# arpg/ba

Hardware: AMD Instinct MI355X
Metric: Gauss-Newton iterations/sec (higher is better)
Workload: dtype f64; 1 GPU; BASELINE.json configs[3]: 10000 poses / 1000000 landmarks / 10000000 reprojection residuals, pinhole, LmSize=1, PoseSize=6, Gauss-Newton (no dogleg), 2 anchor poses inactive; poses=10000, landmarks=1000000, residuals=10000000, reduced_system_n=59988, driver=phase calls of the C-ABI (include/ba_hip.h), parallelism=single GPU

## Files before the change

ba_amd/csrc/k_chol.hip:

```cpp
#include "engine.h"
#include <cstdlib>
#include <algorithm>
#include <vector>

namespace bae {

static const int NB = 64;
static const int LDT = NB + 2;

typedef double double4_t __attribute__((ext_vector_type(4)));

__device__ __forceinline__ double readlane_f64(double v, int lane) {
  int lo = __double2loint(v), hi = __double2hiint(v);
  lo = __builtin_amdgcn_readlane(lo, lane);
  hi = __builtin_amdgcn_readlane(hi, lane);
  return __hiloint2double(hi, lo);
}

static const int LDM = 18;

static const int KC2 = 16;
#ifndef BAE_LDK2
#define BAE_LDK2 (KC2 + 2)
#endif
static const int LDK2 = BAE_LDK2;

__device__ __forceinline__ void update_tile_fast(double* __restrict__ A, uint32_t ld, uint32_t i, uint32_t c,
                                                 uint32_t kb0, uint64_t mask, double (*X)[NB][LDK2],
                                                 double (*Y)[NB][LDK2]) {
  const int tid = threadIdx.x, wave = tid >> 6, lane = tid & 63;
  const int li = lane & 15, lk = lane >> 4;
  const int rb = 32 * (wave >> 1), cb = 32 * (wave & 1);
  double* Aic = A + ((size_t)i * NB) * ld + (size_t)c * NB;
  double4_t acc[2][2];
#pragma unroll
  for (int ti = 0; ti < 2; ++ti)
#pragma unroll
    for (int tj = 0; tj < 2; ++tj) acc[ti][tj] = (double4_t){0.0, 0.0, 0.0, 0.0};
  const int sr = tid >> 3, sc = (tid & 7) * 2;
  const double* Xg0 = A + ((size_t)i * NB + sr) * ld + sc;
  const double* Xg1 = Xg0 + (size_t)32 * ld;
  const double* Yg0 = A + ((size_t)c * NB + sr) * ld + sc;
  const double* Yg1 = Yg0 + (size_t)32 * ld;
  double2 px0[2], px1[2], py0[2], py1[2];
  double F0[4], F1[4];
  double4_t cv[2][2];
#define BAE_SB __builtin_amdgcn_sched_barrier(0)
#define BAE_GLOAD(S, K0)                                        \
  {                                                             \
    px0[S] = *reinterpret_cast<const double2*>(Xg0 + (K0));     \
    px1[S] = *reinterpret_cast<const double2*>(Xg1 + (K0));     \
    py0[S] = *reinterpret_cast<const double2*>(Yg0 + (K0));     \
    py1[S] = *reinterpret_cast<const double2*>(Yg1 + (K0));     \
  }
#define BAE_SSTORE(B, S)                                                    \
  {                                                                         \
    X[B][sr][sc] = px0[S].x; X[B][sr][sc + 1] = px0[S].y;                   \
    X[B][sr + 32][sc] = px1[S].x; X[B][sr + 32][sc + 1] = px1[S].y;         \
    Y[B][sr][sc] = py0[S].x; Y[B][sr][sc + 1] = py0[S].y;                   \
    Y[B][sr + 32][sc] = py1[S].x; Y[B][sr + 32][sc + 1] = py1[S].y;         \
  }
#define BAE_LDF(F, B, KS)                                                              \
  {                                                                                    \
    F[0] = X[B][rb + li][4 * (KS) + lk]; F[1] = X[B][rb + 16 + li][4 * (KS) + lk];     \
    F[2] = Y[B][cb + li][4 * (KS) + lk]; F[3] = Y[B][cb + 16 + li][4 * (KS) + lk];     \
  }
#define BAE_MM(F)                                                                    \
  {                                                                                  \
    acc[0][0] = __builtin_amdgcn_mfma_f64_16x16x4f64(F[0], F[2], acc[0][0], 0, 0, 0); \
    acc[0][1] = __builtin_amdgcn_mfma_f64_16x16x4f64(F[0], F[3], acc[0][1], 0, 0, 0); \
    acc[1][0] = __builtin_amdgcn_mfma_f64_16x16x4f64(F[1], F[2], acc[1][0], 0, 0, 0); \
    acc[1][1] = __builtin_amdgcn_mfma_f64_16x16x4f64(F[1], F[3], acc[1][1], 0, 0, 0); \
  }
#define BAE_CHUNK(J, STORE, LOADK, NEXT)                          \
  {                                                               \
    if (STORE) BAE_SSTORE(((J) + 1) & 1, ((J) + 1) & 1);          \
    LOADK;                                                        \
    BAE_SB; BAE_LDF(F1, (J) & 1, 1); BAE_SB; BAE_MM(F0); BAE_SB;  \
    BAE_LDF(F0, (J) & 1, 2); BAE_SB; BAE_MM(F1); BAE_SB;          \
    BAE_LDF(F1, (J) & 1, 3); BAE_SB; BAE_MM(F0); BAE_SB;          \
    __syncthreads(); BAE_SB;                                      \
    if (NEXT) BAE_LDF(F0, ((J) + 1) & 1, 0);                      \
    BAE_SB; BAE_MM(F1); BAE_SB;                                   \
  }
  uint32_t kcur = (kb0 + (uint32_t)__builtin_ctzll(mask)) * NB;
  mask &= mask - 1;
  BAE_GLOAD(0, kcur);
  BAE_GLOAD(1, kcur + KC2);
  BAE_SSTORE(0, 0);
  BAE_GLOAD(0, kcur + 2 * KC2);
  __syncthreads();
  BAE_LDF(F0, 0, 0);
  while (mask) {
    const uint32_t knext = (kb0 + (uint32_t)__builtin_ctzll(mask)) * NB;
    mask &= mask - 1;
    BAE_CHUNK(0, true, BAE_GLOAD(1, kcur + 3 * KC2), true);
    BAE_CHUNK(1, true, BAE_GLOAD(0, knext), true);
    BAE_CHUNK(2, true, BAE_GLOAD(1, knext + KC2), true);
    BAE_CHUNK(3, true, BAE_GLOAD(0, knext + 2 * KC2), true);
    kcur = knext;
  }
  BAE_CHUNK(0, true, BAE_GLOAD(1, kcur + 3 * KC2), true);
  BAE_CHUNK(1, true, , true);
#define BAE_CLOAD                                                                              \
  _Pragma("unroll") for (int ti = 0; ti < 2; ++ti)                                             \
    _Pragma("unroll") for (int tj = 0; tj < 2; ++tj)                                           \
      _Pragma("unroll") for (int reg = 0; reg < 4; ++reg)                                      \
        cv[ti][tj][reg] = Aic[(size_t)(rb + 16 * ti + lk + 4 * reg) * ld + cb + 16 * tj + li];
  BAE_CHUNK(2, true, BAE_CLOAD, true);
#undef BAE_CLOAD
  BAE_CHUNK(3, false, , false);
#undef BAE_SB
#undef BAE_GLOAD
#undef BAE_SSTORE
#undef BAE_LDF
#undef BAE_MM
#undef BAE_CHUNK
  const bool diag = (i == c);
#pragma unroll
  for (int ti = 0; ti < 2; ++ti)
#pragma unroll
    for (int tj = 0; tj < 2; ++tj)
#pragma unroll
      for (int reg = 0; reg < 4; ++reg) {
        const int r = rb + 16 * ti + lk + 4 * reg;
        const int cc = cb + 16 * tj + li;
        if (!diag || cc <= r) Aic[(size_t)r * ld + cc] = cv[ti][tj][reg] - acc[ti][tj][reg];
      }
}

__device__ __forceinline__ void update_tile(double* __restrict__ A, uint32_t ld, uint32_t nblk, uint32_t i,
                                            uint32_t c, uint32_t kb0, uint32_t kb1,
                                            const double* __restrict__ dsgn, const int* __restrict__ colneg,
                                            const uint8_t* __restrict__ nz, double (*X)[NB][LDK2],
                                            double (*Y)[NB][LDK2], uint32_t* klist) {
  const int rows = (i == nblk) ? 1 : NB;
  const int tid = threadIdx.x, wave = tid >> 6, lane = tid & 63;
  const int li = lane & 15, lk = lane >> 4;
  const int rb = 32 * (wave >> 1), cb = 32 * (wave & 1);
  double* Aic = A + ((size_t)i * NB) * ld + (size_t)c * NB;
  double4_t acc[2][2];
#pragma unroll
  for (int ti = 0; ti < 2; ++ti)
#pragma unroll
    for (int tj = 0; tj < 2; ++tj) acc[ti][tj] = (double4_t){0.0, 0.0, 0.0, 0.0};
  const int sr = tid >> 3, sc = (tid & 7) * 2;
  const double* Xg0 = A + ((size_t)i * NB + (sr < rows ? sr : 0)) * ld + sc;
  const double* Xg1 = A + ((size_t)i * NB + (sr + 32 < rows ? sr + 32 : 0)) * ld + sc;
  const double* Yg0 = A + ((size_t)c * NB + sr) * ld + sc;
  const double* Yg1 = Yg0 + (size_t)32 * ld;
  const double xm0 = sr < rows ? 1.0 : 0.0, xm1 = sr + 32 < rows ? 1.0 : 0.0;
#ifndef BAE_NO_FAST
  if (rows == NB && kb1 - kb0 <= 64u) {
    const uint32_t kl = kb0 + (uint32_t)lane;
    bool on = kl < kb1;
    bool neg = false;
    if (on) {
      neg = colneg[kl] != 0;
      if (nz) on = nz[(size_t)i * nblk + kl] && nz[(size_t)c * nblk + kl];
    }
    const uint64_t mask = __ballot(on);
    if (__ballot(neg) == 0) {
      if (mask == 0) return;
      update_tile_fast(A, ld, i, c, kb0, mask, X, Y);
      return;
    }
  }
#endif
  uint32_t nact = 0;
  for (uint32_t kb = kb0; kb < kb1; ++kb) {
    const bool on = !nz || ((i == nblk || nz[(size_t)i * nblk + kb]) && nz[(size_t)c * nblk + kb]);
    if (on) {
      if (threadIdx.x == 0) klist[nact] = kb * NB;
      ++nact;
    }
  }
  if (nact == 0) return;
  __syncthreads();
  const int nchunk = (int)nact * (NB / KC2);
  double2 px0[2], px1[2], py0[2], py1[2], ps[2] = {make_double2(1.0, 1.0), make_double2(1.0, 1.0)};
  bool plain = rows == NB;
  for (uint32_t kb = kb0; kb < kb1; ++kb) plain = plain && (colneg[kb] == 0);
#define BAE_GLOAD(S, CH)                                                          \
  {                                                                               \
    const uint32_t k0_ = klist[(CH) >> 2] + (uint32_t)((CH) & 3) * KC2;           \
    px0[S] = *reinterpret_cast<const double2*>(Xg0 + k0_);                        \
    px1[S] = *reinterpret_cast<const double2*>(Xg1 + k0_);                        \
    py0[S] = *reinterpret_cast<const double2*>(Yg0 + k0_);                        \
    py1[S] = *reinterpret_cast<const double2*>(Yg1 + k0_);                        \
    if (!plain) ps[S] = *reinterpret_cast<const double2*>(dsgn + k0_ + sc);       \
  }
#define BAE_SSTORE(B, S)                                                          \
  if (plain) {                                                                    \
    X[B][sr][sc] = px0[S].x; X[B][sr][sc + 1] = px0[S].y;                         \
    X[B][sr + 32][sc] = px1[S].x; X[B][sr + 32][sc + 1] = px1[S].y;               \
    Y[B][sr][sc] = py0[S].x; Y[B][sr][sc + 1] = py0[S].y;                         \
    Y[B][sr + 32][sc] = py1[S].x; Y[B][sr + 32][sc + 1] = py1[S].y;               \
  } else {                                                                        \
    X[B][sr][sc] = px0[S].x * xm0; X[B][sr][sc + 1] = px0[S].y * xm0;             \
    X[B][sr + 32][sc] = px1[S].x * xm1; X[B][sr + 32][sc + 1] = px1[S].y * xm1;   \
    Y[B][sr][sc] = ps[S].x * py0[S].x; Y[B][sr][sc + 1] = ps[S].y * py0[S].y;     \
    Y[B][sr + 32][sc] = ps[S].x * py1[S].x; Y[B][sr + 32][sc + 1] = ps[S].y * py1[S].y; \
  }
#define BAE_MMA(B)                                                                \
  _Pragma("unroll") for (int ks = 0; ks < KC2 / 4; ++ks) {                        \
    const double a0 = X[B][rb + li][4 * ks + lk];                                 \
    const double a1 = X[B][rb + 16 + li][4 * ks + lk];                            \
    const double b0 = Y[B][cb + li][4 * ks + lk];                                 \
    const double b1 = Y[B][cb + 16 + li][4 * ks + lk];                            \
    acc[0][0] = __builtin_amdgcn_mfma_f64_16x16x4f64(a0, b0, acc[0][0], 0, 0, 0); \
    acc[0][1] = __builtin_amdgcn_mfma_f64_16x16x4f64(a0, b1, acc[0][1], 0, 0, 0); \
    acc[1][0] = __builtin_amdgcn_mfma_f64_16x16x4f64(a1, b0, acc[1][0], 0, 0, 0); \
    acc[1][1] = __builtin_amdgcn_mfma_f64_16x16x4f64(a1, b1, acc[1][1], 0, 0, 0); \
  }
  BAE_GLOAD(0, 0);
  BAE_GLOAD(1, 1);
  BAE_SSTORE(0, 0);
  BAE_GLOAD(0, 2);
  __syncthreads();
  for (int kc = 0; kc + 2 < nchunk; kc += 2) {
    BAE_SSTORE(1, 1);
    if (kc + 3 < nchunk) BAE_GLOAD(1, kc + 3);
    BAE_MMA(0);
    __syncthreads();
    BAE_SSTORE(0, 0);
    if (kc + 4 < nchunk) BAE_GLOAD(0, kc + 4);
    BAE_MMA(1);
    __syncthreads();
  }
  BAE_SSTORE(1, 1);
  double4_t cv[2][2];
#pragma unroll
  for (int ti = 0; ti < 2; ++ti)
#pragma unroll
    for (int tj = 0; tj < 2; ++tj)
#pragma unroll
      for (int reg = 0; reg < 4; ++reg) {
        const int r = rb + 16 * ti + lk + 4 * reg;
        cv[ti][tj][reg] = Aic[(size_t)(r < rows ? r : 0) * ld + cb + 16 * tj + li];
      }
  BAE_MMA(0);
  __syncthreads();
  BAE_MMA(1);
#undef BAE_GLOAD
#undef BAE_SSTORE
#undef BAE_MMA
  const bool diag = (i == c);
#pragma unroll
  for (int ti = 0; ti < 2; ++ti)
#pragma unroll
    for (int tj = 0; tj < 2; ++tj)
#pragma unroll
      for (int reg = 0; reg < 4; ++reg) {
        const int r = rb + 16 * ti + lk + 4 * reg;
        const int cc = cb + 16 * tj + li;
        if (r < rows && (!diag || cc <= r)) Aic[(size_t)r * ld + cc] = cv[ti][tj][reg] - acc[ti][tj][reg];
      }
}

template <bool BULK>
__global__ void __launch_bounds__(256, BULK ? 2 : 4)
k_update2(double* __restrict__ A, uint32_t ld, uint32_t nblk, uint32_t c0, uint32_t kb0,
          uint32_t kb1, const double* __restrict__ dsgn, const int* __restrict__ colneg, int swz,
          const uint8_t* __restrict__ nz, const OwnMap own) {
  __shared__ double X[2][NB][LDK2];
  __shared__ double Y[2][NB][LDK2];
  __shared__ uint32_t klist[32];
  __shared__ double pad_[BULK ? 2432 : 1];
  if (BULK && kb0 == 0xffffffffu) pad_[threadIdx.x] = 0.0;
  if (!BULK) __builtin_amdgcn_s_setprio(2);
  uint32_t c, i;
  if (swz & 1) {
    const uint32_t sbl = (uint32_t)swz >> 8;
    const uint32_t b = blockIdx.x, xcd = b & 7u, slot = b >> 3;
    const uint32_t t = (slot >> (2 * sbl)) * 8u + xcd, within = slot & ((1u << (2 * sbl)) - 1u);
    uint32_t sr = (uint32_t)((sqrt(8.0 * (double)t + 1.0) - 1.0) * 0.5);
    while ((uint64_t)(sr + 1) * (sr + 2) / 2 <= t) ++sr;
    while ((uint64_t)sr * (sr + 1) / 2 > t) --sr;
    const uint32_t sc = t - (uint32_t)((uint64_t)sr * (sr + 1) / 2);
    const uint32_t R = (sr << sbl) + (within >> sbl), C = (sc << sbl) + (within & ((1u << sbl) - 1u));
    if (C > R) return;
    c = c0 + C;
    i = c0 + R;
    if (i > nblk || c >= nblk) return;
  } else {
    c = c0 + blockIdx.y;
    i = c + blockIdx.x;
    if (i > nblk) return;
  }
  if (!own_tile(own, i, c, nblk)) return;
  update_tile(A, ld, nblk, i, c, kb0, kb1, dsgn, colneg, nz, X, Y, klist);
}

static const int NB2 = 128;
#ifdef BAE_TIME128
__device__ unsigned long long* g_t128_buf = nullptr;
__device__ unsigned int g_t128_n = 0;
static const unsigned int T128_CAP = 1u << 21, T128_REC = 6;
#endif
template <bool RECT, bool LIST = false>
__global__ void __launch_bounds__(256, 2)
k_update128(double* __restrict__ A, uint32_t ld, uint32_t nblk, uint32_t c0, uint32_t m2, uint32_t kb0,
            uint32_t kb1, const double* __restrict__ dsgn, const int* __restrict__ colneg, uint32_t sbl,
            const uint8_t* __restrict__ nz, const OwnMap own,
            uint32_t nrow64, uint32_t r0, uint32_t rect_cols) {
  __shared__ double X[2][NB2][LDK2];
  __shared__ double Y[2][NB2][LDK2];
  __shared__ uint32_t klist[32];
  if (blockIdx.x < nrow64) {
    const uint32_t mcols = RECT ? 2 * rect_cols : nblk - c0, y = blockIdx.x / mcols;
    const uint32_t c = c0 + blockIdx.x % mcols, i = nblk - y;
    if (y > ((nblk - r0) & 1u) || c > i || c >= nblk) return;
    if (!own_tile(own, i, c, nblk)) return;
    update_tile(A, ld, nblk, i, c, kb0, kb1, dsgn, colneg, nz, reinterpret_cast<double(*)[NB][LDK2]>(&X[0][0][0]),
                reinterpret_cast<double(*)[NB][LDK2]>(&Y[0][0][0]), klist);
    return;
  }
  const uint32_t b = blockIdx.x - nrow64;
  uint32_t R, C;
  if constexpr (LIST) {
    const uint32_t gb = own.G >> 1, per = gb * gb;
    const uint32_t pr = b / per, within = b - pr * per;
    const uint2* pairs = reinterpret_cast<const uint2*>(((unsigned long long)own.pairs_hi << 32) | own.pairs_lo);
    const uint2 bp = pairs[pr];
    const uint32_t base = c0 / own.G;
    R = (bp.x - base) * gb + within / gb;
    C = (bp.y - base) * gb + within % gb;
    if (C > R || R >= m2) return;
  } else if (RECT) {
    R = b / rect_cols;
    C = b % rect_cols;
    if (R >= m2) return;
  } else {
    const uint32_t xcd = b & 7u, slot = b >> 3;
    const uint32_t t = (slot >> (2 * sbl)) * 8u + xcd, within = slot & ((1u << (2 * sbl)) - 1u);
    uint32_t sr_ = (uint32_t)((sqrt(8.0 * (double)t + 1.0) - 1.0) * 0.5);
    while ((uint64_t)(sr_ + 1) * (sr_ + 2) / 2 <= t) ++sr_;
    while ((uint64_t)sr_ * (sr_ + 1) / 2 > t) --sr_;
    const uint32_t sc_ = t - (uint32_t)((uint64_t)sr_ * (sr_ + 1) / 2);
    R = (sr_ << sbl) + (within >> sbl);
    C = (sc_ << sbl) + (within & ((1u << sbl) - 1u));
    if (C > R || R >= m2) return;
  }
  const uint32_t c = c0 + 2 * C, i = r0 + 2 * R;
  if (!own_tile(own, i, c, nblk)) return;
  const int tid = threadIdx.x, wave = tid >> 6, lane = tid & 63;
  const uint32_t kl = kb0 + (uint32_t)lane;
  bool on = kl < kb1, neg = false;
  if (on) {
    neg = colneg[kl] != 0;
    if (nz)
      on = (nz[(size_t)i * nblk + kl] | nz[(size_t)(i + 1) * nblk + kl]) &&
           (nz[(size_t)c * nblk + kl] | nz[(size_t)(c + 1) * nblk + kl]);
  }
  uint64_t mask = __ballot(on);
  if (mask == 0) return;
  if (__ballot(neg) != 0 || kb1 - kb0 > 64u) {
    double(*X64)[NB][LDK2] = reinterpret_cast<double(*)[NB][LDK2]>(&X[0][0][0]);
    double(*Y64)[NB][LDK2] = reinterpret_cast<double(*)[NB][LDK2]>(&Y[0][0][0]);
    for (uint32_t q = 0; q < 4; ++q) {
      const uint32_t ii = i + (q >> 1), cc = c + (q & 1);
      if (cc > ii) continue;
      __syncthreads();
      update_tile(A, ld, nblk, ii, cc, kb0, kb1, dsgn, colneg, nz, X64, Y64, klist);
    }
    return;
  }
  const bool diag = (i == c);
  const int li = lane & 15, lk = lane >> 4;
  const int rb = 64 * (wave >> 1), cb = 64 * (wave & 1);
  double4_t acc[4][4];
#pragma unroll
  for (int ti = 0; ti < 4; ++ti)
#pragma unroll
    for (int tj = 0; tj < 4; ++tj) acc[ti][tj] = (double4_t){0.0, 0.0, 0.0, 0.0};
  const int sr = tid >> 3, sc = (tid & 7) * 2;
  const double* Xg = A + ((size_t)i * NB + sr) * ld + sc;
  const double* Yg = A + ((size_t)c * NB + sr) * ld + sc;
  const size_t ld32 = (size_t)32 * ld;
  double2 px[4], py[4];
  double FA0[4], FB0[4], FA1[4], FB1[4];
#ifdef BAE_NO_SCHED_PINS_128
#define BAE_SB
#else
#define BAE_SB __builtin_amdgcn_sched_barrier(0)
#endif
#ifndef BAE_KMASK
#define BAE_KMASK 0xffffffffu
#endif
#define BAE_GLOAD(K0)                                                                \
  _Pragma("unroll") for (int u = 0; u < 4; ++u) {                                    \
    px[u] = *reinterpret_cast<const double2*>(Xg + u * ld32 + ((K0) & BAE_KMASK));   \
    py[u] = *reinterpret_cast<const double2*>(Yg + u * ld32 + ((K0) & BAE_KMASK));   \
  }
#define BAE_SSTORE(B)                                                                \
  _Pragma("unroll") for (int u = 0; u < 4; ++u) {                                    \
    X[B][sr + 32 * u][sc] = px[u].x; X[B][sr + 32 * u][sc + 1] = px[u].y;            \
    Y[B][sr + 32 * u][sc] = py[u].x; Y[B][sr + 32 * u][sc + 1] = py[u].y;            \
  }
#define BAE_LDF(FA, FB, B, KS)                                                       \
  _Pragma("unroll") for (int q = 0; q < 4; ++q) {                                    \
    FA[q] = X[B][rb + 16 * q + li][4 * (KS) + lk];                                   \
    FB[q] = Y[B][cb + 16 * q + li][4 * (KS) + lk];                                   \
  }
#define BAE_MM(FA, FB)                                                               \
  _Pragma("unroll") for (int ti = 0; ti < 4; ++ti)                                   \
    _Pragma("unroll") for (int tj = 0; tj < 4; ++tj)                                 \
      acc[ti][tj] = __builtin_amdgcn_mfma_f64_16x16x4f64(FA[ti], FB[tj], acc[ti][tj], 0, 0, 0);
#define BAE_CHUNK(J, STORE, LOADK, NEXT)                                             \
  {                                                                                  \
    if (STORE) BAE_SSTORE(((J) + 1) & 1);                                            \
    LOADK;                                                                           \
    BAE_SB; BAE_LDF(FA1, FB1, (J) & 1, 1); BAE_SB; BAE_MM(FA0, FB0); BAE_SB;         \
    BAE_LDF(FA0, FB0, (J) & 1, 2); BAE_SB; BAE_MM(FA1, FB1); BAE_SB;                 \
    BAE_LDF(FA1, FB1, (J) & 1, 3); BAE_SB; BAE_MM(FA0, FB0); BAE_SB;                 \
    __syncthreads(); BAE_SB;                                                         \
    if (NEXT) BAE_LDF(FA0, FB0, ((J) + 1) & 1, 0);                                   \
    BAE_SB; BAE_MM(FA1, FB1); BAE_SB;                                                \
  }
#ifdef BAE_TIME128
  const unsigned long long tt0 = __builtin_readcyclecounter();
  const unsigned long long tw0 = wall_clock64();
  const int tt_cols = __builtin_popcountll(mask);
#endif
  uint32_t kcur = (kb0 + (uint32_t)__builtin_ctzll(mask)) * NB;
  mask &= mask - 1;
  BAE_GLOAD(kcur);
  BAE_SSTORE(0);
  BAE_GLOAD(kcur + KC2);
  __syncthreads();
  BAE_LDF(FA0, FB0, 0, 0);
#ifdef BAE_TIME128
  const unsigned long long tt1 = __builtin_readcyclecounter();
  const unsigned long long tw1 = wall_clock64();
#endif
  while (mask) {
    const uint32_t knext = (kb0 + (uint32_t)__builtin_ctzll(mask)) * NB;
    mask &= mask - 1;
    BAE_CHUNK(0, true, BAE_GLOAD(kcur + 2 * KC2), true);
    BAE_CHUNK(1, true, BAE_GLOAD(kcur + 3 * KC2), true);
    BAE_CHUNK(2, true, BAE_GLOAD(knext), true);
    BAE_CHUNK(3, true, BAE_GLOAD(knext + KC2), true);
    kcur = knext;
  }
  double* Aic = A + ((size_t)i * NB) * ld + (size_t)c * NB;
  double4_t cva[4], cvb[4];
#define BAE_CLOAD(CV, TI)                                                            \
  _Pragma("unroll") for (int tj = 0; tj < 4; ++tj)                                   \
    _Pragma("unroll") for (int reg = 0; reg < 4; ++reg)                              \
      CV[tj][reg] = Aic[(size_t)(rb + 16 * (TI) + lk + 4 * reg) * ld + cb + 16 * tj + li];
#define BAE_CSTORE(CV, TI)                                                           \
  _Pragma("unroll") for (int tj = 0; tj < 4; ++tj)                                   \
    _Pragma("unroll") for (int reg = 0; reg < 4; ++reg) {                            \
      const int r = rb + 16 * (TI) + lk + 4 * reg;                                   \
      const int cc = cb + 16 * tj + li;                                              \
      if (!diag || cc <= r) Aic[(size_t)r * ld + cc] = CV[tj][reg] - acc[TI][tj][reg]; \
    }
  BAE_CHUNK(0, true, BAE_GLOAD(kcur + 2 * KC2), true);
  BAE_CHUNK(1, true, BAE_GLOAD(kcur + 3 * KC2), true);
  BAE_CHUNK(2, true, , true);
  BAE_CHUNK(3, false, BAE_CLOAD(cva, 0), false);
#ifdef BAE_TIME128
  const unsigned long long tt2 = __builtin_readcyclecounter();
  const unsigned long long tw2 = wall_clock64();
#endif
  if (diag && wave == 1) return;
  BAE_SB;
  BAE_CLOAD(cvb, 1);
  BAE_SB;
  BAE_CSTORE(cva, 0);
  BAE_SB;
  BAE_CLOAD(cva, 2);
  BAE_SB;
  BAE_CSTORE(cvb, 1);
  BAE_SB;
  BAE_CLOAD(cvb, 3);
  BAE_SB;
  BAE_CSTORE(cva, 2);
  BAE_CSTORE(cvb, 3);
#ifdef BAE_TIME128
  if (tid == 0 && (blockIdx.x % 257u) == 100u && !RECT) {
    const unsigned long long tt3 = __builtin_readcyclecounter();
    printf("T128 cols %d prologue %llu loop %llu epilogue %llu per_chunk %llu loop_100MHz %llu\n", tt_cols, tt1 - tt0,
           tt2 - tt1, tt3 - tt2, (tt2 - tt1) / (unsigned long long)(4 * tt_cols), tw2 - tw1);
  }
  if (tid == 0 && !RECT && g_t128_buf) {
    const unsigned int idx = atomicAdd(&g_t128_n, 1u);
    if (idx < T128_CAP) {
      unsigned long long* r = g_t128_buf + (size_t)idx * T128_REC;
      r[0] = tw0; r[1] = tw1; r[2] = tw2; r[3] = wall_clock64();
      r[4] = ((unsigned long long)__builtin_amdgcn_s_getreg(6164) << 32) | (unsigned int)__builtin_amdgcn_s_getreg(63492);
      r[5] = (unsigned long long)blockIdx.x | ((unsigned long long)tt_cols << 32) | ((unsigned long long)kb0 << 40);
    }
  }
#endif
#undef BAE_CLOAD
#undef BAE_CSTORE
#undef BAE_SB
#undef BAE_GLOAD
#undef BAE_SSTORE
#undef BAE_LDF
#undef BAE_MM
#undef BAE_CHUNK
}

static const int NOPV = 40;

struct TileLds {
  double T[NB][LDT];
  double Md[4][16][LDM];
  double dv[NB];
  double sg[NB];
  __attribute__((aligned(16))) double colbuf[2][NB];
  int bad;
  int neg;
};

__device__ __forceinline__ void factor_tile_wave0(TileLds& sh, int lane, const double* __restrict__ floor_tile) {
  const int li = lane & 15, lk = lane >> 4;
  unsigned long long negmask = 0;
#pragma unroll
  for (int pb = 0; pb < 4; ++pb) {
    const int c0 = 16 * pb;
    double p[16];
#pragma unroll
    for (int c = 0; c < 16; ++c) p[c] = (c0 + c <= lane) ? sh.T[lane][c0 + c] : 0.0;
    double sa_prev = 0.0;
    double lb[16];
    double d = readlane_f64(p[0], c0);
#pragma unroll
    for (int j = 0; j < 16; ++j) {
      const int J = c0 + j;
      const int dhi = __double2hiint(d);
      const int sbit = dhi & (int)0x80000000;
      negmask |= (unsigned long long)((unsigned)dhi >> 31) << J;
      const double ad = fabs(d);
#define BAE_UPD(n)                                      \
  {                                                     \
    const int c_ = j + 1 + (n);                         \
    if (j > 0 && c_ < 16) p[c_] -= sa_prev * lb[c_];    \
  }
#define BAE_SB __builtin_amdgcn_sched_barrier(0)
      double y = __builtin_amdgcn_rsq(ad);
      BAE_SB;
      double t = ad * y;
      BAE_SB;
      double h = fma(-t, y, 1.0);
      BAE_UPD(0) BAE_SB;
      double q = fma(0.375, h, 0.5);
      double yh = y * h;
      BAE_UPD(1) BAE_UPD(2) BAE_UPD(3) BAE_SB;
      y = fma(yh, q, y);
      BAE_UPD(4) BAE_UPD(5) BAE_UPD(6) BAE_UPD(7) BAE_UPD(8) BAE_SB;
      const double sa = p[j] * y;
      BAE_UPD(9) BAE_UPD(10) BAE_SB;
      const double l = __hiloint2double(__double2hiint(sa) ^ sbit, __double2loint(sa));
      sh.colbuf[j & 1][lane] = l;
      p[j] = l;
      BAE_UPD(11) BAE_UPD(12) BAE_UPD(13) BAE_UPD(14) BAE_SB;
#pragma unroll
      for (int c = j + 2; c < 16; ++c) lb[c] = sh.colbuf[j & 1][c0 + c];
      BAE_SB;
      if (j < 15) {
        p[j + 1] -= sa * readlane_f64(l, J + 1);
        d = readlane_f64(p[j + 1], J + 1);
      }
      BAE_SB;
#undef BAE_UPD
#undef BAE_SB
      sa_prev = sa;
    }
#pragma unroll
    for (int c = 0; c < 16; ++c) sh.T[lane][c0 + c] = (c0 + c <= lane) ? p[c] : 0.0;
    sh.sg[lane] = ((negmask >> lane) & 1ull) ? -1.0 : 1.0;
    if (pb < 3) {
      double la[4][3], nb[4][3];
#pragma unroll
      for (int ks = 0; ks < 4; ++ks) {
        const int k = c0 + 4 * ks + lk;
        const double sk = -sh.sg[k];
#pragma unroll
        for (int b = pb + 1; b < 4; ++b) {
          la[ks][b - 1] = sh.T[16 * b + li][k];
          nb[ks][b - 1] = sk * la[ks][b - 1];
        }
      }
#pragma unroll
      for (int rbk = pb + 1; rbk < 4; ++rbk)
#pragma unroll
        for (int cbk = pb + 1; cbk <= rbk; ++cbk) {
          double4_t acc;
#pragma unroll
          for (int reg = 0; reg < 4; ++reg) acc[reg] = sh.T[16 * rbk + lk + 4 * reg][16 * cbk + li];
#pragma unroll
          for (int ks = 0; ks < 4; ++ks)
            acc = __builtin_amdgcn_mfma_f64_16x16x4f64(la[ks][rbk - 1], nb[ks][cbk - 1], acc, 0, 0, 0);
#pragma unroll
          for (int reg = 0; reg < 4; ++reg) sh.T[16 * rbk + lk + 4 * reg][16 * cbk + li] = acc[reg];
        }
    }
  }
  if (lane == 0) sh.neg = negmask != 0 ? 1 : 0;
  {
    const double q = sh.T[lane][lane];
    if (!(q > 0.0 && q < 1e150)) sh.bad = 1;
    if (floor_tile && q * q < floor_tile[lane]) sh.bad = 1;
    sh.dv[lane] = 1.0 / q;
  }
  {
    const int base = 16 * lk, c = li;
    double sacc[16];
#pragma unroll
    for (int r = 0; r < 16; ++r) sacc[r] = (r == c) ? 1.0 : 0.0;
#pragma unroll
    for (int k = 0; k < 16; ++k) {
      const double xk = sacc[k] * sh.dv[base + k];
      sacc[k] = xk;
#pragma unroll
      for (int r = k + 1; r < 16; ++r) sacc[r] -= sh.T[base + r][base + k] * xk;
    }
#pragma unroll
    for (int r = 0; r < 16; ++r) sh.Md[lk][r][c] = sacc[r];
  }
}

__device__ __forceinline__ double subst_operand(const TileLds& sh, int v, int li, int lk, bool sgn) {
  if (v < 16) {
    const int c = v >> 2, ks = v & 3;
    return (sgn ? sh.sg[16 * c + li] : 1.0) * sh.Md[c][li][4 * ks + lk];
  }
  const int pi = (v - 16) >> 2, ks = v & 3;
  const int c = pi == 0 ? 1 : (pi < 3 ? 2 : 3);
  const int k = pi == 0 ? 0 : (pi < 3 ? pi - 1 : pi - 3);
  const int kk = 16 * k + 4 * ks + lk;
  return -(sgn ? sh.sg[kk] : 1.0) * sh.T[16 * c + li][kk];
}

__device__ __forceinline__ void subst_rows(double4_t R[4], const double op[NOPV]) {
#pragma unroll
  for (int c = 0; c < 4; ++c) {
    double4_t Zc = (double4_t){0.0, 0.0, 0.0, 0.0};
#pragma unroll
    for (int ks = 0; ks < 4; ++ks) Zc = __builtin_amdgcn_mfma_f64_16x16x4f64(op[4 * c + ks], R[c][ks], Zc, 0, 0, 0);
#pragma unroll
    for (int c2 = c + 1; c2 < 4; ++c2) {
      const int pi = (c2 == 1 ? 0 : (c2 == 2 ? 1 : 3)) + c;
#pragma unroll
      for (int ks = 0; ks < 4; ++ks)
        R[c2] = __builtin_amdgcn_mfma_f64_16x16x4f64(op[16 + 4 * pi + ks], Zc[ks], R[c2], 0, 0, 0);
    }
    R[c] = Zc;
  }
}

template <bool FACTOR>
__global__ void __launch_bounds__(256, 2)
k_step_update(double* __restrict__ A, uint32_t ld, uint32_t nblk, uint32_t c0, uint32_t kb0,
              uint32_t kb1, double* __restrict__ dsgn, double* __restrict__ opbuf,
              int* __restrict__ colneg, int* __restrict__ status, const uint8_t* __restrict__ nz,
              uint32_t row_end, const uint32_t* __restrict__ rowlist) {
  struct UpdLds { double X[2][NB][LDK2]; double Y[2][NB][LDK2]; };
  __shared__ uint32_t klist[32];
  constexpr size_t kLds = sizeof(TileLds) > sizeof(UpdLds) ? sizeof(TileLds) : sizeof(UpdLds);
  __shared__ __attribute__((aligned(16))) unsigned char smem[kLds];
  UpdLds& u = *reinterpret_cast<UpdLds*>(smem);
  TileLds& sh = *reinterpret_cast<TileLds*>(smem);
  __builtin_amdgcn_s_setprio(2);
  const uint32_t c = c0 + blockIdx.y;
  const uint32_t i = rowlist ? rowlist[blockIdx.x] : c + blockIdx.x;
  if (i > nblk || i >= row_end || i < c) return;
  const bool special = FACTOR && (i == c0 && c == c0);
  if (!special) {
    update_tile(A, ld, nblk, i, c, kb0, kb1, dsgn, colneg, nz, u.X, u.Y, klist);
    return;
  }
  const int rows = (i == nblk) ? 1 : NB;
  const int tid = threadIdx.x, wave = tid >> 6, lane = tid & 63;
  const int li = lane & 15, lk = lane >> 4;
  const int rb = 32 * (wave >> 1), cb = 32 * (wave & 1);
  uint32_t nact = 0;
  for (uint32_t kb = kb0; kb < kb1; ++kb) {
    const bool on = !nz || ((i == nblk || nz[(size_t)i * nblk + kb]) && nz[(size_t)c * nblk + kb]);
    if (on) {
      if (tid == 0) klist[nact] = kb * NB;
      ++nact;
    }
  }
  __syncthreads();
  double* Aic = A + ((size_t)i * NB) * ld + (size_t)c * NB;
  double4_t acc[2][2];
#pragma unroll
  for (int ti = 0; ti < 2; ++ti)
#pragma unroll
    for (int tj = 0; tj < 2; ++tj)
#pragma unroll
      for (int reg = 0; reg < 4; ++reg) {
        const int r = rb + 16 * ti + lk + 4 * reg;
        acc[ti][tj][reg] = Aic[(size_t)(r < rows ? r : 0) * ld + cb + 16 * tj + li];
      }
  const int nchunk = (int)nact * (NB / KC2);
  if (nchunk > 0) {
    const int sr = tid >> 3, sc = (tid & 7) * 2;
    const double* Xg0 = A + ((size_t)i * NB + (sr < rows ? sr : 0)) * ld + sc;
    const double* Xg1 = A + ((size_t)i * NB + (sr + 32 < rows ? sr + 32 : 0)) * ld + sc;
    const double* Yg0 = A + ((size_t)c * NB + sr) * ld + sc;
    const double* Yg1 = Yg0 + (size_t)32 * ld;
    const double xm0 = sr < rows ? 1.0 : 0.0, xm1 = sr + 32 < rows ? 1.0 : 0.0;
    double2 px0, px1, py0, py1, ps;
    auto gload = [&](uint32_t k0) {
      px0 = *reinterpret_cast<const double2*>(Xg0 + k0);
      px1 = *reinterpret_cast<const double2*>(Xg1 + k0);
      py0 = *reinterpret_cast<const double2*>(Yg0 + k0);
      py1 = *reinterpret_cast<const double2*>(Yg1 + k0);
      ps = *reinterpret_cast<const double2*>(dsgn + k0 + sc);
    };
    auto sstore = [&](int b) {
      u.X[b][sr][sc] = px0.x * xm0; u.X[b][sr][sc + 1] = px0.y * xm0;
      u.X[b][sr + 32][sc] = px1.x * xm1; u.X[b][sr + 32][sc + 1] = px1.y * xm1;
      u.Y[b][sr][sc] = -ps.x * py0.x; u.Y[b][sr][sc + 1] = -ps.y * py0.y;
      u.Y[b][sr + 32][sc] = -ps.x * py1.x; u.Y[b][sr + 32][sc + 1] = -ps.y * py1.y;
    };
    auto kof = [&](int ch) { return klist[ch >> 2] + (uint32_t)(ch & 3) * KC2; };
    gload(kof(0));
    sstore(0);
    if (nchunk > 1) gload(kof(1));
    __syncthreads();
    for (int kc = 0; kc < nchunk; ++kc) {
      const int b = kc & 1;
      if (kc + 1 < nchunk) sstore(b ^ 1);
      if (kc + 2 < nchunk) gload(kof(kc + 2));
#pragma unroll
      for (int ks = 0; ks < KC2 / 4; ++ks) {
        const double a0 = u.X[b][rb + li][4 * ks + lk];
        const double a1 = u.X[b][rb + 16 + li][4 * ks + lk];
        const double b0 = u.Y[b][cb + li][4 * ks + lk];
        const double b1 = u.Y[b][cb + 16 + li][4 * ks + lk];
        acc[0][0] = __builtin_amdgcn_mfma_f64_16x16x4f64(a0, b0, acc[0][0], 0, 0, 0);
        acc[0][1] = __builtin_amdgcn_mfma_f64_16x16x4f64(a0, b1, acc[0][1], 0, 0, 0);
        acc[1][0] = __builtin_amdgcn_mfma_f64_16x16x4f64(a1, b0, acc[1][0], 0, 0, 0);
        acc[1][1] = __builtin_amdgcn_mfma_f64_16x16x4f64(a1, b1, acc[1][1], 0, 0, 0);
      }
      __syncthreads();
    }
  }
  __builtin_amdgcn_s_setprio(3);
#pragma unroll
  for (int ti = 0; ti < 2; ++ti)
#pragma unroll
    for (int tj = 0; tj < 2; ++tj)
#pragma unroll
      for (int reg = 0; reg < 4; ++reg) {
        const int r = rb + 16 * ti + lk + 4 * reg;
        const int cc = cb + 16 * tj + li;
        sh.T[r][cc] = (cc <= r) ? acc[ti][tj][reg] : 0.0;
      }
  if (tid == 0) sh.bad = 0;
  __syncthreads();
  const double* floors = *reinterpret_cast<const double* const*>(status + 2);
  if (wave == 0) factor_tile_wave0(sh, lane, floors ? floors + (size_t)c0 * NB : nullptr);
  __syncthreads();
  {
    double* ob = opbuf + (size_t)c0 * NOPV * 64;
#pragma unroll
    for (int q = 0; q < NOPV / 4; ++q) {
      const int v = wave * (NOPV / 4) + q;
      ob[(size_t)v * 64 + lane] = subst_operand(sh, v, li, lk, true);
    }
    if (tid < NB) dsgn[(size_t)c0 * NB + tid] = sh.sg[tid];
    if (tid == 0) colneg[c0] = sh.neg;
    if (tid == 0 && sh.bad) atomicExch(status, 1);
  }
}

__global__ void __launch_bounds__(256)
k_trsm_op(double* __restrict__ A, uint32_t ld, uint32_t d, uint32_t nblk,
          const double* __restrict__ opbuf, const uint8_t* __restrict__ nz, const uint32_t* __restrict__ rowlist) {
  __builtin_amdgcn_s_setprio(3);
  const int tid = threadIdx.x, wave = tid >> 6, lane = tid & 63;
  const int li = lane & 15, lk = lane >> 4;
  const uint32_t i = rowlist ? rowlist[blockIdx.x] : d + 1 + blockIdx.x;
  if (nz && i < nblk && !nz[(size_t)i * nblk + d]) return;
  const int rows = (i == nblk) ? 1 : NB;
  const int myrow = 16 * wave + li;
  double* Xrow = A + ((size_t)i * NB + (myrow < rows ? myrow : 0)) * ld + (size_t)d * NB;
  double4_t R[4];
#pragma unroll
  for (int c = 0; c < 4; ++c)
#pragma unroll
    for (int reg = 0; reg < 4; ++reg) R[c][reg] = Xrow[16 * c + lk + 4 * reg];
  double op[NOPV];
  const double* ob = opbuf + (size_t)d * NOPV * 64 + lane;
#pragma unroll
  for (int v = 0; v < NOPV; ++v) op[v] = ob[(size_t)v * 64];
  subst_rows(R, op);
  if (myrow < rows) {
#pragma unroll
    for (int c = 0; c < 4; ++c)
#pragma unroll
      for (int reg = 0; reg < 4; ++reg) Xrow[16 * c + lk + 4 * reg] = R[c][reg];
  }
}

struct SquareLds {
  TileLds t;
  double X[3][NB][LDT];
// ... 1355 lines not shown
```

Before: 1.740 iterations/sec.

## Interleave LDS fragment reads and global loads between individual MFMAs in Cholesky update

```diff
diff --git a/ba_amd/csrc/k_chol.hip b/ba_amd/csrc/k_chol.hip
--- a/ba_amd/csrc/k_chol.hip
+++ b/ba_amd/csrc/k_chol.hip
@@ -324,8 +324,8 @@
     const uint2* pairs = reinterpret_cast<const uint2*>(((unsigned long long)own.pairs_hi << 32) | own.pairs_lo);
     const uint2 bp = pairs[pr];
     const uint32_t base = c0 / own.G;
-    R = (bp.x - base) * gb + within / gb;
-    C = (bp.y - base) * gb + within % gb;
+    R = __builtin_amdgcn_readfirstlane((bp.x - base) * gb + within / gb);
+    C = __builtin_amdgcn_readfirstlane((bp.y - base) * gb + within % gb);
     if (C > R || R >= m2) return;
   } else if (RECT) {
     R = b / rect_cols;
@@ -375,9 +375,11 @@
 #pragma unroll
     for (int tj = 0; tj < 4; ++tj) acc[ti][tj] = (double4_t){0.0, 0.0, 0.0, 0.0};
   const int sr = tid >> 3, sc = (tid & 7) * 2;
-  const double* Xg = A + ((size_t)i * NB + sr) * ld + sc;
-  const double* Yg = A + ((size_t)c * NB + sr) * ld + sc;
-  const size_t ld32 = (size_t)32 * ld;
+  const char* Xrow = reinterpret_cast<const char*>(A + (size_t)i * NB * ld);
+  const char* Yrow = reinterpret_cast<const char*>(A + (size_t)c * NB * ld);
+  uint32_t voff[4];
+#pragma unroll
+  for (int u = 0; u < 4; ++u) voff[u] = (((uint32_t)sr + 32u * u) * ld + (uint32_t)sc) * 8u;
   double2 px[4], py[4];
   double FA0[4], FB0[4], FA1[4], FB1[4];
 #ifdef BAE_NO_SCHED_PINS_128
@@ -388,35 +390,49 @@
 #ifndef BAE_KMASK
 #define BAE_KMASK 0xffffffffu
 #endif
+#define BAE_VOFF_PIN asm volatile("" : "+v"(voff[0]), "+v"(voff[1]), "+v"(voff[2]), "+v"(voff[3]))
+#define BAE_GLOAD1(P, ROW, U, K0)                                                    \
+  P[U] = *reinterpret_cast<const double2*>(ROW + (size_t)((K0) & BAE_KMASK) * sizeof(double) + (size_t)voff[U]);
+#define BAE_SSTORE1(S, P, B, U)                                                      \
+  { S[B][sr + 32 * (U)][sc] = P[U].x; S[B][sr + 32 * (U)][sc + 1] = P[U].y; }
 #define BAE_GLOAD(K0)                                                                \
   _Pragma("unroll") for (int u = 0; u < 4; ++u) {                                    \
-    px[u] = *reinterpret_cast<const double2*>(Xg + u * ld32 + ((K0) & BAE_KMASK));   \
-    py[u] = *reinterpret_cast<const double2*>(Yg + u * ld32 + ((K0) & BAE_KMASK));   \
+    BAE_GLOAD1(px, Xrow, u, K0) BAE_GLOAD1(py, Yrow, u, K0)                          \
   }
 #define BAE_SSTORE(B)                                                                \
   _Pragma("unroll") for (int u = 0; u < 4; ++u) {                                    \
-    X[B][sr + 32 * u][sc] = px[u].x; X[B][sr + 32 * u][sc + 1] = px[u].y;            \
-    Y[B][sr + 32 * u][sc] = py[u].x; Y[B][sr + 32 * u][sc + 1] = py[u].y;            \
+    BAE_SSTORE1(X, px, B, u) BAE_SSTORE1(Y, py, B, u)                                \
+  }
+#define BAE_LDF1(FA, FB, B, KS, Q)                                                   \
+  {                                                                                  \
+    if ((Q) == 0 || (Q) >= 5) {                                                      \
+      const int q_ = (Q) == 0 ? 0 : (Q) - 4;                                         \
+      FA[q_] = X[B][rb + 16 * q_ + li][4 * (KS) + lk];                               \
+    } else {                                                                         \
+      FB[(Q) - 1] = Y[B][cb + 16 * ((Q) - 1) + li][4 * (KS) + lk];                   \
+    }                                                                                \
   }
 #define BAE_LDF(FA, FB, B, KS)                                                       \
-  _Pragma("unroll") for (int q = 0; q < 4; ++q) {                                    \
-    FA[q] = X[B][rb + 16 * q + li][4 * (KS) + lk];                                   \
-    FB[q] = Y[B][cb + 16 * q + li][4 * (KS) + lk];                                   \
-  }
-#define BAE_MM(FA, FB)                                                               \
-  _Pragma("unroll") for (int ti = 0; ti < 4; ++ti)                                   \
-    _Pragma("unroll") for (int tj = 0; tj < 4; ++tj)                                 \
-      acc[ti][tj] = __builtin_amdgcn_mfma_f64_16x16x4f64(FA[ti], FB[tj], acc[ti][tj], 0, 0, 0);
-#define BAE_CHUNK(J, STORE, LOADK, NEXT)                                             \
-  {                                                                                  \
-    if (STORE) BAE_SSTORE(((J) + 1) & 1);                                            \
-    LOADK;                                                                           \
-    BAE_SB; BAE_LDF(FA1, FB1, (J) & 1, 1); BAE_SB; BAE_MM(FA0, FB0); BAE_SB;         \
-    BAE_LDF(FA0, FB0, (J) & 1, 2); BAE_SB; BAE_MM(FA1, FB1); BAE_SB;                 \
-    BAE_LDF(FA1, FB1, (J) & 1, 3); BAE_SB; BAE_MM(FA0, FB0); BAE_SB;                 \
-    __syncthreads(); BAE_SB;                                                         \
-    if (NEXT) BAE_LDF(FA0, FB0, ((J) + 1) & 1, 0);                                   \
-    BAE_SB; BAE_MM(FA1, FB1); BAE_SB;                                                \
+  _Pragma("unroll") for (int q = 0; q < 8; ++q) BAE_LDF1(FA, FB, B, KS, q)
+#define BAE_STEP(CA, CB, READ, NA, NBF, RB, RKS, SP, S, P, ROW, SB, STORE, LOAD, K0)             \
+  _Pragma("unroll") for (int t = 0; t < 16; ++t) {                                               \
+    acc[t >> 2][t & 3] = __builtin_amdgcn_mfma_f64_16x16x4f64(CA[t >> 2], CB[t & 3], acc[t >> 2][t & 3], 0, 0, 0); \
+    if ((READ) && t < 8) BAE_LDF1(NA, NBF, RB, RKS, t)                                           \
+    if ((SP) && t >= 8 && (t & 1) == 0) {                                                        \
+      if (STORE) BAE_SSTORE1(S, P, SB, (t - 8) >> 1)                                             \
+      if (LOAD) BAE_GLOAD1(P, ROW, (t - 8) >> 1, K0)                                             \
+    }                                                                                            \
+    BAE_SB;                                                                                      \
+  }
+#define BAE_CHUNK(J, STORE, LOAD, K0, NEXT, PRE)                                                           \
+  {                                                                                                        \
+    PRE;                                                                                                   \
+    BAE_SB;                                                                                                \
+    BAE_STEP(FA0, FB0, true, FA1, FB1, (J) & 1, 1, true, X, px, Xrow, ((J) + 1) & 1, STORE, LOAD, K0)      \
+    BAE_STEP(FA1, FB1, true, FA0, FB0, (J) & 1, 2, true, Y, py, Yrow, ((J) + 1) & 1, STORE, LOAD, K0)      \
+    BAE_STEP(FA0, FB0, true, FA1, FB1, (J) & 1, 3, false, X, px, Xrow, 0, false, false, 0)                 \
+    __syncthreads(); BAE_SB;                                                                               \
+    BAE_STEP(FA1, FB1, NEXT, FA0, FB0, ((J) + 1) & 1, 0, false, X, px, Xrow, 0, false, false, 0)           \
   }
 #ifdef BAE_TIME128
   const unsigned long long tt0 = __builtin_readcyclecounter();
@@ -437,10 +453,11 @@
   while (mask) {
     const uint32_t knext = (kb0 + (uint32_t)__builtin_ctzll(mask)) * NB;
     mask &= mask - 1;
-    BAE_CHUNK(0, true, BAE_GLOAD(kcur + 2 * KC2), true);
-    BAE_CHUNK(1, true, BAE_GLOAD(kcur + 3 * KC2), true);
-    BAE_CHUNK(2, true, BAE_GLOAD(knext), true);
-    BAE_CHUNK(3, true, BAE_GLOAD(knext + KC2), true);
+    BAE_VOFF_PIN;
+    BAE_CHUNK(0, true, true, kcur + 2 * KC2, true, );
+    BAE_CHUNK(1, true, true, kcur + 3 * KC2, true, );
+    BAE_CHUNK(2, true, true, knext, true, );
+    BAE_CHUNK(3, true, true, knext + KC2, true, );
     kcur = knext;
   }
   double* Aic = A + ((size_t)i * NB) * ld + (size_t)c * NB;
@@ -456,10 +473,11 @@
       const int cc = cb + 16 * tj + li;                                              \
       if (!diag || cc <= r) Aic[(size_t)r * ld + cc] = CV[tj][reg] - acc[TI][tj][reg]; \
     }
-  BAE_CHUNK(0, true, BAE_GLOAD(kcur + 2 * KC2), true);
-  BAE_CHUNK(1, true, BAE_GLOAD(kcur + 3 * KC2), true);
-  BAE_CHUNK(2, true, , true);
-  BAE_CHUNK(3, false, BAE_CLOAD(cva, 0), false);
+  BAE_VOFF_PIN;
+  BAE_CHUNK(0, true, true, kcur + 2 * KC2, true, );
+  BAE_CHUNK(1, true, true, kcur + 3 * KC2, true, );
+  BAE_CHUNK(2, true, false, 0, true, );
+  BAE_CHUNK(3, false, false, 0, false, BAE_CLOAD(cva, 0));
 #ifdef BAE_TIME128
   const unsigned long long tt2 = __builtin_readcyclecounter();
   const unsigned long long tw2 = wall_clock64();
@@ -500,7 +518,11 @@
 #undef BAE_GLOAD
 #undef BAE_SSTORE
 #undef BAE_LDF
-#undef BAE_MM
+#undef BAE_GLOAD1
+#undef BAE_VOFF_PIN
+#undef BAE_SSTORE1
+#undef BAE_LDF1
+#undef BAE_STEP
 #undef BAE_CHUNK
 }
 
```

After: 1.765 iterations/sec (median of 6 runs). 1.4% higher.
